# ikt-luh/Demo-Learned-Point-Cloud-Compression

Hardware: AMD Instinct MI355X
Metric: point-cloud frames/sec encode+decode @1M pts (higher is better)
Workload: dtype f32

## Files before the change

### demo-learned-point-cloud-compression_amd/csrc/codec.hip

```cpp
#include "common.h"

#include <string.h>

#include <algorithm>
#include <atomic>
#include <chrono>
#include <deque>
#include <exception>
#include <new>
#include <map>
#include <memory>
#include <string>
#include <condition_variable>
#include <functional>
#include <mutex>
#include <thread>
#include <vector>

namespace {

double now_s() {
  return std::chrono::duration<double>(std::chrono::steady_clock::now().time_since_epoch()).count();
}

// ... 1868 lines not shown
    slots.resize((size_t)n_frames);
    for (int f = 0; f < n_frames; ++f) {
      const int32_t pl = r.be32();
      for (int s = 0; s < 3; ++s) ks[s].push_back(r.be32());
      slots[f] = {r.bytes(pl), pl};
      PCC_REQUIRE(!r.bad, PCC_E_STREAM, "pcc_decode_gop: truncated container");
    }
    if (!v1 && len - r.pos >= 8 && memcmp(h_in + r.pos, "PCSK", 4) == 0) {
      Reader t{h_in + r.pos + 4, len - r.pos - 4};
      const int32_t cnt = t.be32();
      bool ok = cnt >= 1 && cnt <= 63 && (int64_t)cnt * 16 <= t.len - t.pos;
      for (int k = 0; ok && k < cnt; ++k) {
        const int64_t i = t.be32();
        const uint64_t hi = (uint32_t)t.be32(), lo = (uint32_t)t.be32();
        const int64_t w = t.be32();
        ok = !t.bad && i > (sk_idx.empty() ? 0 : sk_idx.back()) && i < (int64_t)ny_hdr * cy && w >= 2 && w * 4 <= ylen &&
             ((hi << 32) | lo) >= ((uint64_t)1 << 31);
        sk_idx.push_back(i);
        sk_state.push_back((hi << 32) | lo);
        sk_word.push_back(w);
      }
      if (!ok) sk_idx.clear();
    }
    return PCC_OK;
  }
  int check_sizes() {
    fn.assign((size_t)n_frames, 0);
    fdepth.assign((size_t)n_frames, 0);
    for (int f = 0; f < n_frames; ++f) {
      int32_t org[3];
      PCC_TRY(pcc_octree_peek(slots[f].p, slots[f].len, &fn[f], &fdepth[f], org));
      PCC_REQUIRE(fn[f] >= 0 && fn[f] <= ((int64_t)slots[f].len + 64) * 4096, PCC_E_STREAM,
                  "pcc_decode_gop: frame %d announces %lld points in a %d-byte blob", f, (long long)fn[f], slots[f].len);
      if (fn[f] > 0) {
        const int d = fdepth[f];
        PCC_REQUIRE(d >= 1 && d <= 13, PCC_E_STREAM, "pcc_decode_gop: frame %d: octree depth %d", f, d);
        for (int a = 0; a < 3; ++a) {
          const int64_t biased = (int64_t)org[a] + 4096;
          PCC_REQUIRE(biased >= 0 && biased + ((int64_t)1 << d) <= 8192 && (biased & (((int64_t)1 << d) - 1)) == 0,
                      PCC_E_STREAM, "pcc_decode_gop: frame %d: octree origin %d (axis %d) is not on the 2^%d grid", f,
                      org[a], a, d);
        }
      }
      ny += fn[f];
    }
    PCC_REQUIRE(ny == ny_hdr, PCC_E_STREAM, "pcc_decode_gop: container says N_y=%d, geometry gives %lld", ny_hdr,
                (long long)ny);
    PCC_REQUIRE(nz_hdr <= ny_hdr, PCC_E_STREAM, "pcc_decode_gop: container says N_z=%d > N_y=%d", nz_hdr, ny_hdr);
    PCC_REQUIRE(ny_hdr <= kMaxLatentRows, PCC_E_STREAM, "pcc_decode_gop: container says N_y=%d, this build decodes at most %lld",
                ny_hdr, (long long)kMaxLatentRows);
    return PCC_OK;
  }
  void start_z_job() {
    zsym.resize((size_t)std::max<int64_t>((int64_t)nz_hdr * cz, 1));
    cd->workers.run(0, [this]() {
      if (nz_hdr == 0) return;
      if (cd->eb_tables && cz <= 256) {
        std::vector<uint8_t> idx8((size_t)nz_hdr * cz);
        for (int c = 0; c < cz; ++c) memset(idx8.data() + (size_t)c * nz_hdr, c, (size_t)nz_hdr);
        z_rc = pcc_rans_decode8_gated(zstr, zlen, idx8.data(), (int64_t)nz_hdr * cz, eb_cdf->i32(), (int)eb_cdf->dims[1],
                                      eb_len->i32(), eb_off->i32(), (int)eb_cdf->dims[0], zsym.data(), nullptr, cd->eb_tables);
        if (z_rc != PCC_OK) z_err = pcc_last_error();
        return;
      }
      std::vector<int32_t> idx((size_t)nz_hdr * cz);
      for (int c = 0; c < cz; ++c) std::fill(idx.begin() + (size_t)c * nz_hdr, idx.begin() + (size_t)(c + 1) * nz_hdr, c);
      z_rc = pcc_rans_decode(zstr, zlen, idx.data(), (int64_t)nz_hdr * cz, eb_cdf->i32(), (int)eb_cdf->dims[1],
                             eb_len->i32(), eb_off->i32(), (int)eb_cdf->dims[0], zsym.data());
      if (z_rc != PCC_OK) z_err = pcc_last_error();
    });
  }
  int start_z() {
    eb_cdf = find(cd, "entropy_bottleneck.quantized_cdf");
    eb_len = find(cd, "entropy_bottleneck.cdf_length");
    eb_off = find(cd, "entropy_bottleneck.offset");
    PCC_REQUIRE(eb_cdf && eb_len && eb_off, PCC_E_ARG, "pcc_decode_gop: entropy_bottleneck tables missing");
    cd->workers.ensure(1);
    z_early = !v1 && (int64_t)nz_hdr * cz <= kEarlyZSymbols;
    if (z_early) start_z_job();
    if (!v1) return PCC_OK;
    int64_t zn = 0, yn = 0;
    PCC_TRY(pcc_rans_stream_info(zstr, zlen, &zn, &z_steps, &z_chunks));
    PCC_TRY(pcc_rans_stream_info(ystr, ylen, &yn, &y_steps, &y_chunks));
    PCC_REQUIRE(zn == (int64_t)nz_hdr * cz && yn == (int64_t)ny_hdr * cy, PCC_E_STREAM,
                "pcc_decode_gop: streams hold %lld / %lld symbols, header says %lld / %lld", (long long)yn, (long long)zn,
                (long long)ny_hdr * cy, (long long)nz_hdr * cz);
    d_status = (int32_t*)cd->pool.alloc(4);
    if (!d_status) return PCC_E_NOMEM;
    PCC_HIP(hipMemsetAsync(d_status, 0, 4, st));
    PCC_TRY(cd->pin_dec.ensure((size_t)ylen + (size_t)zlen + 512));
    memcpy(cd->pin_dec.p, zstr, (size_t)zlen);
    memcpy(cd->pin_dec.p + (((size_t)zlen + 255) & ~(size_t)255), ystr, (size_t)ylen);
    if ((int64_t)nz_hdr * cz <= kEarlyZSymbols) return z_stream_dev(&zsym_early);
    return PCC_OK;
  }
  int z_stream_dev(int32_t** zs) {
    const size_t zpad = ((size_t)zlen + 255) & ~(size_t)255;
    CODEC_ALLOC(d_str, uint8_t, zpad + (size_t)ylen + 256);
    if (!*zs) *zs = (int32_t*)cd->pool.alloc(sizeof(int32_t) * (size_t)(std::max<int64_t>((int64_t)nz_hdr, 1) * cz));
    if (!*zs) return PCC_E_NOMEM;
    PCC_HIP(hipMemcpyAsync(d_str, cd->pin_dec.p, zpad + (size_t)ylen, hipMemcpyHostToDevice, st));
    d_ystr = d_str + zpad;
    return pcc_rans_decode_dev(ctx, cd->eb_dev, d_str, zlen, (int64_t)nz_hdr * cz, z_steps, z_chunks, nullptr,
                               std::max<int64_t>(nz_hdr, 1), *zs, d_status);
  }
  int geometry() {
    std::vector<std::vector<int32_t>> fpts((size_t)n_frames);
    PCC_TRY(cd->pin_keys.ensure((size_t)std::max<int64_t>(ny, 1) * 16));
    int32_t* yc_h = (int32_t*)cd->pin_keys.p;
    std::vector<int64_t> frow((size_t)n_frames + 1, 0);
    for (int f = 0; f < n_frames; ++f) frow[(size_t)f + 1] = frow[(size_t)f] + fn[f];
    std::vector<PartJob> pjobs;
    std::vector<int> fpart0((size_t)n_frames, -1), fparts((size_t)n_frames, 0);
    for (int f = 0; f < n_frames; ++f) {
      if (fn[f] == 0 || slots[f].p[1] != 3) continue;
      int K = 0;
      const uint8_t* pp[16];
      int64_t pl[16];
      PCC_TRY(pcc_octree_parts(slots[f].p, slots[f].len, &K, pp, pl));
      int32_t org[3];
      PCC_TRY(pcc_octree_peek(slots[f].p, slots[f].len, nullptr, nullptr, org));
      fpart0[f] = (int)pjobs.size();
      fparts[f] = K;
      int64_t row = frow[(size_t)f];
      for (int k = 0; k < K; ++k) {
        int64_t n = 0;
        PCC_TRY(pcc_octree_peek(pp[k], pl[k], &n, nullptr, nullptr));
        pjobs.push_back({f, k, pp[k], pl[k], n, row, {org[0], org[1], org[2]}});
        row += n;
      }
    }
    constexpr int kPartThreads = 8;
    const int nj = (int)pjobs.size();
    if (nj > 0) cd->workers.ensure(kPartThreads);
    for (int j0 = 0; j0 < nj; j0 += kPartThreads) {
      const int j1 = std::min(nj, j0 + kPartThreads);
      for (int j = j0 + 1; j < j1; ++j) cd->workers.run(j - j0, [&pjobs, yc_h, j]() { run_part_job(pjobs[(size_t)j], yc_h); });
      run_part_job(pjobs[(size_t)j0], yc_h);
      cd->workers.wait_range(1, kPartThreads);
    }
    for (const PartJob& pj : pjobs)
      if (pj.rc != PCC_OK) {
        pcc_set_error("pcc_decode_gop (geometry, frame %d part %d): %s", pj.f, pj.k, pj.err.c_str());
        return pj.rc;
      }
    bool out_of_range = false;
    for (int f = 0; f < n_frames; ++f) {
      if (fn[f] == 0) continue;
      int64_t level_n[16];
      if (slots[f].p[1] == 3) {
        for (int L = 0; L < 16; ++L) level_n[L] = 0;
        bool any = false;
        uint64_t last = 0;
        int64_t total = 0;
        for (int k = 0; k < fparts[f]; ++k) {
          const PartJob& pj = pjobs[(size_t)(fpart0[f] + k)];
          out_of_range |= pj.out_of_range;
          if (pj.out.cells.empty()) continue;
          PCC_REQUIRE(!any || (pj.out.cells.front() >> 6) > (last >> 6), PCC_E_STREAM,
                      "pcc_decode_gop: frame %d: part %d begins inside or in front of the cell the part before it ends in", f, k);
          any = true;
          last = pj.out.cells.back();
          total += (int64_t)pj.out.cells.size();
          for (int L = 0; L < 16; ++L) level_n[L] += pj.out.level_n[L];
        }
        PCC_REQUIRE(total == fn[f], PCC_E_STREAM, "pcc_decode_gop: frame %d decoded %lld points, announced %lld", f, (long long)total,
                    (long long)fn[f]);
      } else {
        if (slots[f].p[1] == 2) {
          int64_t n2 = 0;
          fpts[f].resize((size_t)(3 * fn[f]));
          PCC_TRY(pcc_octree2_decode(ctx, slots[f].p, slots[f].len, nullptr, fpts[f].data(), fn[f], &n2, level_n));
        } else {
          PCC_TRY(pcc_octree_unpack_vec(slots[f].p, slots[f].len, &fpts[f], level_n));
        }
        PCC_REQUIRE((int64_t)fpts[f].size() == 3 * fn[f], PCC_E_STREAM, "pcc_decode_gop: frame %d decoded %zu points, announced %lld",
                    f, fpts[f].size() / 3, (long long)fn[f]);
        out_of_range |= put_leaf_rows(fpts[f].data(), fn[f], f, yc_h + 4 * frow[(size_t)f]);
      }
      const int depth = fdepth[f];
      n16 += depth >= 1 ? level_n[depth - 1] : 1;
      n32 += depth >= 2 ? level_n[depth - 2] : 1;
      n_batch = f + 1;
    }
    if (!z_early && !v1) start_z_job();
    PCC_REQUIRE(!out_of_range && n_batch <= 65535, PCC_E_RANGE, "pcc_decode_gop: decoded coordinate out of range");
    return PCC_OK;
  }
  int z_decode() {
    std::vector<int64_t> y_level_n(2, 0);
    CODEC_ALLOC(yc, int32_t, 4 * std::max<int64_t>(ny, 1));
    CODEC_ALLOC(keys, uint64_t, std::max<int64_t>(ny, 1));
    CODEC_ALLOC(flag, int32_t, 1);
    CODEC_ALLOC(perm, uint32_t, std::max<int64_t>(ny, 1));
    if (ny > 0) {
      PCC_HIP(hipMemcpyAsync(yc, cd->pin_keys.p, (size_t)ny * 16, hipMemcpyHostToDevice, st));
      PCC_HIP(hipMemsetAsync(flag, 0, 4, st));
      PCC_TRY(pcc_morton_keys(ctx, yc, ny, keys, flag));
      PCC_TRY(pcc_sort_pairs(ctx, keys, perm, ny, 0));
      y_level_n[0] = n16;
      y_level_n[1] = n32;
    }
    ycs = new_set(cd, keys, ny, 8, std::max(n_batch, 1));
    if (ny > 0) ycs->down_counts = y_level_n;
    PCC_TRY(down_of(cd, ycs));
    PCC_TRY(down_of(cd, ycs->down));
    CS* zcs = ycs->down->down;
    View zv;
    PCC_TRY(view_of(cd, zcs, &zv));
    PCC_REQUIRE(zcs->n == nz_hdr, PCC_E_STREAM, "pcc_decode_gop: container says N_z=%d, coordinates give %lld", nz_hdr,
                (long long)zcs->n);
    PCC_TRY(view_of(cd, ycs, &yv));
    {
      CS *a_cs, *pre_cs;
      PCC_TRY(up_of(cd, zcs, &a_cs));
      PCC_TRY(up_of(cd, a_cs, &pre_cs));
      PCC_TRY(h_s_book_at(cd, pre_cs, ycs, yv, &hs_book));
    }
    cd->workers.wait_all();
    if (z_rc != PCC_OK) {
      pcc_set_error("pcc_decode_gop (z stream): %s", z_err.c_str());
      return z_rc;
    }
    const int64_t nz = zcs->n;
    CODEC_ALLOC(zsym_d_own, int32_t, std::max<int64_t>(nz, 1) * cz);
    int32_t* zsym_d = zsym_d_own;
    CODEC_ALLOC(rows, float, std::max<int64_t>(nz, 1) * cz);
    if (v1) {
      if (zsym_early)
        zsym_d = zsym_early;
      else
        PCC_TRY(z_stream_dev(&zsym_d));
      if (nz > 0) PCC_TRY(pcc_factorized_dequant(ctx, zsym_d, nz, cz, cd->dev["entropy_bottleneck.medians"], rows));
    } else if (nz > 0) {
      PCC_TRY(cd->pin_zsym.ensure((size_t)nz * cz * 4));
      memcpy(cd->pin_zsym.p, zsym.data(), (size_t)nz * cz * 4);
      PCC_HIP(hipMemcpyAsync(zsym_d, cd->pin_zsym.p, (size_t)nz * cz * 4, hipMemcpyHostToDevice, st));
      PCC_TRY(pcc_factorized_dequant(ctx, zsym_d, nz, cz, cd->dev["entropy_bottleneck.medians"], rows));
    }
    float* zf;
    PCC_TRY(rows_to_tensor(cd, zv, rows, cz, &zf));
    z_hat = {zcs, zf, cz};
    return PCC_OK;
  }
  int y_decode() {
    float* params;
    PCC_TRY(h_s_out_at(cd, gp, ycs, yv, &params, hs_book));
    float* scale_d;
    const double q_dec[2] = {qg, qa};
    PCC_TRY(scale_rows_dev(cd, 1, q_dec, 1, &scale_d));
    const Tensor* tab = find(cd, "gaussian_conditional.scale_table");
    const Tensor *gc_cdf = find(cd, "gaussian_conditional.quantized_cdf"), *gc_len = find(cd, "gaussian_conditional.cdf_length"),
                 *gc_off = find(cd, "gaussian_conditional.offset");
    const Tensor* ab = find(cd, "entropy_model.offsets_ab");
    PCC_REQUIRE(tab && gc_cdf && gc_len && gc_off && ab, PCC_E_ARG, "pcc_decode_gop: gaussian_conditional tables missing");
    const int64_t tot = (int64_t)cy * ny;
    CODEC_ALLOC(idx8, uint8_t, std::max<int64_t>(tot, 1));
    CODEC_ALLOC(sym_d, int32_t, std::max<int64_t>(tot, 1));
    CODEC_ALLOC(rows, float, std::max<int64_t>(tot, 1));
    if (ny > 0 && v1) {
      PCC_TRY(pcc_gaussian_indexes8(ctx, params, ny, cy, scale_d, cd->dev["gaussian_conditional.scale_table"],
                                    (int)tab->dims[0], idx8));
      PCC_TRY(pcc_rans_decode_dev(ctx, cd->gc_dev, d_ystr, ylen, tot, y_steps, y_chunks, idx8, 1, sym_d, d_status));
      PCC_TRY(pcc_gaussian_dequant(ctx, sym_d, params, ny, cy, scale_d, tab->f32()[0], ab->f32()[0], ab->f32()[1], rows));
    } else if (ny > 0) {
      PCC_TRY(pcc_gaussian_indexes8(ctx, params, ny, cy, scale_d, cd->dev["gaussian_conditional.scale_table"],
                                    (int)tab->dims[0], idx8));
      PCC_TRY(cd->pin_yidx.ensure((size_t)tot));
      PCC_TRY(cd->pin_dec.ensure((size_t)tot * 4));
      PCC_HIP(hipMemcpyAsync(cd->pin_yidx.p, idx8, (size_t)tot, hipMemcpyDeviceToHost, st));
      PCC_HIP(hipStreamSynchronize(st));
      {
        CS* c0;
        int32_t* nbr0;
        PCC_TRY(up_of(cd, ycs, &c0));
        PCC_TRY(nbr27_of(cd, pcc_conv_up_fused() ? ycs : c0, &nbr0));
      }
      bool decoded = false;
      if (!sk_idx.empty() && cd->gc_tables) {
        const int pieces = (int)sk_idx.size() + 1;
        std::vector<int> prc((size_t)pieces, PCC_OK);
        std::vector<uint64_t> end_x((size_t)pieces, 0);
        std::vector<int64_t> end_w((size_t)pieces, 0);
        auto piece = [&](int k) {
          const int64_t lo = k == 0 ? 0 : sk_idx[k - 1], hi = k == pieces - 1 ? tot : sk_idx[k];
          prc[k] = pcc_rans_decode8_range(ystr, ylen, cd->pin_yidx.p, tot, gc_cdf->i32(), (int)gc_cdf->dims[1], gc_len->i32(),
                                          gc_off->i32(), (int)gc_cdf->dims[0], (int32_t*)cd->pin_dec.p, cd->gc_tables, lo, hi,
                                          k == 0 ? 0 : sk_state[k - 1], k == 0 ? 0 : sk_word[k - 1], &end_x[k], &end_w[k]);
        };
        {
          WorkersGuard wait_pieces{&cd->workers};
          cd->workers.ensure(pieces - 1);
          for (int k = 1; k < pieces; ++k) cd->workers.run(k - 1, [&piece, k]() { piece(k); });
          piece(0);
        }
        decoded = true;
        for (int k = 0; k < pieces; ++k) {
          decoded &= prc[k] == PCC_OK;
          if (k + 1 < pieces) decoded &= end_x[k] == sk_state[k] && end_w[k] == sk_word[k];
        }
        if (decoded)
          PCC_HIP(hipMemcpyAsync(sym_d, cd->pin_dec.p, (size_t)tot * 4, hipMemcpyHostToDevice, st));
      }
      const int n_chunks = tot >= (1 << 16) ? 4 : 1;
      std::vector<int64_t> bound((size_t)n_chunks);
      for (int c = 0; c < n_chunks; ++c) bound[c] = c == n_chunks - 1 ? tot : (tot * (c + 1) / n_chunks) & ~(int64_t)63;
      struct UpUser {
        const int64_t* bound;
        const uint8_t* host;
        int32_t* dev;
        hipStream_t st;
        bool failed;
      } up{bound.data(), cd->pin_dec.p, sym_d, st, false};
      PccRansGate gate{n_chunks, bound.data(),
                       [](void* u, int c) {
                         UpUser* g = (UpUser*)u;
                         const int64_t lo = c == 0 ? 0 : g->bound[c - 1], hi = g->bound[c];
                         if (hi > lo && hipMemcpyAsync(g->dev + lo, g->host + (size_t)lo * 4, (size_t)(hi - lo) * 4,
                                                       hipMemcpyHostToDevice, g->st) != hipSuccess)
                           g->failed = true;
                       },
                       &up};
      if (!decoded)
        PCC_TRY(pcc_rans_decode8_gated(ystr, ylen, cd->pin_yidx.p, tot, gc_cdf->i32(), (int)gc_cdf->dims[1],
                                       gc_len->i32(), gc_off->i32(), (int)gc_cdf->dims[0], (int32_t*)cd->pin_dec.p,
                                       &gate, cd->gc_tables));
      PCC_REQUIRE(!up.failed, PCC_E_HIP, "pcc_decode_gop: hipMemcpyAsync of decoded symbols failed");
      PCC_TRY(pcc_gaussian_dequant(ctx, sym_d, params, ny, cy, scale_d, tab->f32()[0], ab->f32()[0], ab->f32()[1], rows));
    }
    float* yf;
    PCC_TRY(rows_to_tensor(cd, yv, rows, cy, &yf));
    y_hat = {ycs, yf, cy};
    return PCC_OK;
  }
  int synthesis(const PackedDst* dst) {
    Feat h = y_hat;
    const int nb = h.cs->n_batch;
    {
      const std::vector<int64_t>* o0;
      PCC_TRY(offsets_of(cd, h.cs, &o0));
    }
    const float* rgb_cand = nullptr;
    bool tail = false;
    uint64_t* tail_pkeys = nullptr;
    int tail_shift = 0;
    for (int j = 0; j < 3; ++j) {
      const std::string uname = "g_s.up" + std::to_string(j);
      const std::string cname = "g_s.conv" + std::to_string(j), oname = "g_s.occ" + std::to_string(j);
      const float *w, *b, *hw, *hb;
      const Tensor *tw, *thw;
      PCC_TRY(wb(cd, cname, &w, &b, &tw));
      PCC_TRY(wb(cd, oname, &hw, &hb, &thw));
      const int cin = (int)tw->dims[1], cout = (int)tw->dims[2];
      const bool fused = pcc_conv_up_fused() && cin == 32 && cout == 32 && cd->dev.count(uname + ".weight#perm");
      Feat u;
      PCC_TRY(up2(cd, uname, h, 1, &u, fused));
      const int64_t nu = u.cs->n;
      const Tensor* tcol = find(cd, "g_s.color.weight");
      const bool with_rgb = fused && j == 2 && nu > 0 && tcol && tcol->dims.size() == 2 && tcol->dims[0] == 32 &&
                            tcol->dims[1] == 3;
      float* feats = nullptr;
      if (!with_rgb) {
        feats = (float*)cd->pool.alloc(sizeof(float) * (size_t)(std::max<int64_t>(nu, 1) * cout));
        if (!feats) return PCC_E_NOMEM;
      }
      CODEC_ALLOC(logits, float, std::max<int64_t>(nu, 1));
      if (with_rgb) {
        int32_t* pn;
        PCC_TRY(nbr27_of(cd, h.cs, &pn));
        CODEC_ALLOC(rgb_all, float, nu * 3);
        rgb_cand = rgb_all;
        PCC_TRY(pcc_sparse_conv_head_up_perm_rgb(ctx, u.f, h.cs->n, pn, h.cs->n, w, b, 1, hw, hb, logits,
                                                 cd->dev["g_s.color.weight"], cd->dev["g_s.color.bias"], rgb_all));
      } else if (fused && nu > 0) {
        int32_t* pn;
        PCC_TRY(nbr27_of(cd, h.cs, &pn));
        PCC_TRY(pcc_sparse_conv_head_up_perm(ctx, u.f, h.cs->n, pn, h.cs->n, w, b, 1, feats, hw, hb, logits));
      } else if (nu == 0) {
      } else {
        int32_t* nbr;
        PCC_TRY(nbr27_of(cd, u.cs, &nbr));
        PCC_TRY(pcc_sparse_conv_head(ctx, u.f, nu, nbr, 27, nu, nu, w, b, cin, cout, 1, feats, hw, hb, logits));
      }
      const std::vector<int64_t>* offs;
      PCC_TRY(offsets_of(cd, u.cs, &offs));
      std::vector<int64_t> kj((size_t)nb), new_offs(1, 0);
      for (int f = 0; f < nb; ++f) {
        const int64_t want = f < (int)ks[j].size() ? ks[j][f] : 0;
        kj[f] = std::max<int64_t>(0, std::min<int64_t>(want, (*offs)[f + 1] - (*offs)[f]));
        new_offs.push_back(new_offs.back() + kj[f]);
      }
      CODEC_ALLOC(keep, uint32_t, std::max<int64_t>(nu, 1));
      const int64_t n_keep = new_offs.back();
      int32_t* keep_remap = nullptr;
      if (nu > 0 && j + 1 < 3) {
        keep_remap = (int32_t*)cd->pool.alloc(sizeof(int32_t) * (size_t)nu);
        if (!keep_remap) return PCC_E_NOMEM;
      }
      if (nu > 0) PCC_TRY(pcc_topk_prune_map(ctx, logits, nu, nb, offs->data(), kj.data(), keep, nullptr, keep_remap));
      CODEC_ALLOC(pkeys, uint64_t, std::max<int64_t>(n_keep, 1));
      CODEC_ALLOC(pf, float, std::max<int64_t>(n_keep, 1) * cout);
      const bool in_place = cout == 32;
      tail = with_rgb && in_place && n_keep > 0 && !u.cs->keys && u.cs->gen_parent;
      if (tail) {
        PCC_TRY(keys_of(cd, u.cs->gen_parent, &tail_pkeys));
        tail_shift = 3 * log2i(u.cs->stride);
        pkeys = nullptr;
      } else if (n_keep > 0) {
        if (!u.cs->keys && u.cs->gen_parent) {
          uint64_t* pk;
          PCC_TRY(keys_of(cd, u.cs->gen_parent, &pk));
          PCC_TRY(pcc_up_coords_rows(ctx, pk, u.cs->gen_parent->n, 3 * log2i(u.cs->stride), keep, n_keep, pkeys));
        } else {
          PCC_TRY(pcc_gather_rows(ctx, u.cs->keys, keep, n_keep, 8, pkeys));
        }
        if (!in_place) PCC_TRY(pcc_gather_rows(ctx, feats, keep, n_keep, 4 * cout, pf));
      }
      CS* ps = new_set(cd, pkeys, n_keep, u.cs->stride, nb);
      ps->offsets = new_offs;
      ps->subset_of = u.cs;
      ps->keep = keep;
      ps->keep_remap = keep_remap;
      h = {ps, in_place ? feats : pf, cout, in_place ? keep : nullptr};
    }
    {
      const float *w, *b;
      const Tensor* tw;
      PCC_TRY(wb(cd, "g_s.color", &w, &b, &tw));
      const int64_t nr = h.cs->n;
      CODEC_ALLOC(rgb, float, std::max<int64_t>(nr, 1) * 3);
      CODEC_ALLOC(coords, int32_t, std::max<int64_t>(nr, 1) * 4);
      cd->rec_xyz16 = nullptr;
      cd->rec_rgbp = nullptr;
      if (nr > 0 && tail && rgb_cand && h.rows) {
        if (dst && nr <= dst->cap) {
          CODEC_ALLOC(xyz16, int16_t, nr * 3);
          CODEC_ALLOC(rgbp, float, nr * 3);
          cd->rec_xyz16 = xyz16;
          cd->rec_rgbp = rgbp;
        }
        hipLaunchKernelGGL(k_decode_tail, dim3((unsigned)((nr + 255) / 256)), dim3(256), 0, st, (const uint64_t*)tail_pkeys,
                           tail_shift, h.rows, nr, rgb_cand, (int4*)coords, rgb, cd->rec_xyz16, cd->rec_rgbp);
        PCC_CHECK_LAUNCH();
      } else if (nr > 0) {
        if (rgb_cand && h.rows)
          PCC_TRY(pcc_gather_rows(ctx, rgb_cand, h.rows, nr, 12, rgb));
        else if (h.rows && (int)tw->dims[0] == 32 && (int)tw->dims[1] <= 8)
          PCC_TRY(pcc_linear_gather(ctx, h.f, h.rows, nr, w, b, (int)tw->dims[1], 0, rgb));
        else if (h.rows) {
          CODEC_ALLOC(pf, float, nr * h.c);
          PCC_TRY(pcc_gather_rows(ctx, h.f, h.rows, nr, 4 * h.c, pf));
          PCC_TRY(pcc_linear(ctx, pf, nr, w, b, (int)tw->dims[0], (int)tw->dims[1], 0, rgb));
        } else
          PCC_TRY(pcc_linear(ctx, h.f, nr, w, b, (int)tw->dims[0], (int)tw->dims[1], 0, rgb));
        uint64_t* hkeys;
        PCC_TRY(keys_of(cd, h.cs, &hkeys));
        PCC_TRY(pcc_keys_to_coords(ctx, hkeys, nr, coords));
      }
      cd->rec_coords = coords;
      cd->rec_i16 = true;
      cd->rec_colors = rgb;
      cd->rec_n = nr;
      cd->rec_offsets = h.cs->offsets;
    }
    return finish(dst);
  }
  int finish(const PackedDst* dst) {
    if (v1) {
      PCC_TRY(cd->pin_flag.ensure(64));
      PCC_HIP(hipMemcpyAsync(cd->pin_flag.p, d_status, 4, hipMemcpyDeviceToHost, st));
    }
    if (dst && cd->rec_n > 0) {
      PCC_REQUIRE(cd->rec_n <= dst->cap && dst->points && dst->colors, PCC_E_ARG,
                  "pcc_decode_gop_packed: %lld points decoded, destination holds %lld", (long long)cd->rec_n,
                  (long long)dst->cap);
      PCC_TRY(queue_packed(cd, dst->points, dst->colors));
    }
    PCC_TRY(pcc_sync(ctx));
    if (dst && cd->rec_n > 0) {
      cd->workers.wait_all();
      PCC_REQUIRE(cd->widen_status.load() == 0, PCC_E_HIP, "pcc_decode_gop_packed: wait for the points' copy failed");
    }
    if (v1 && *(volatile int32_t*)cd->pin_flag.p != 0) {
      cd->rec_n = 0;
      cd->rec_offsets.clear();
      pcc_set_error("pcc_decode_gop: malformed interleaved rANS stream (status %d)", *(int32_t*)cd->pin_flag.p);
      return PCC_E_STREAM;
    }
    return PCC_OK;
  }
};

}

static int decode_gop_impl(pcc_codec* cd, const uint8_t* h_in, int64_t len, pcc_cloud_info* h_info,
                           double* h_stage_s, const PackedDst* dst = nullptr) {
  PCC_REQUIRE(cd && cd->ctx, PCC_E_ARG, "pcc_decode_gop: null codec");
  PCC_REQUIRE(h_in && len >= 36 && h_info, PCC_E_STREAM, "pcc_decode_gop: container shorter than its header");
  PCC_TRY(begin_call(cd));
  cd->rec_n = 0;
  cd->rec_offsets.clear();
  cd->rec_i16 = false;
  cd->rec_xyz16 = nullptr;
  cd->rec_rgbp = nullptr;
  DecodeCall c(cd);
  PCC_TRY(timed(&c.ts[0], [&] { return c.parse(h_in, len); }));
  PCC_TRY(c.check_sizes());
  WorkersGuard z_job{&cd->workers};
  PCC_TRY(c.start_z());
  PCC_TRY(timed(&c.ts[1], [&] { return c.geometry(); }));
  PCC_TRY(timed(&c.ts[2], [&] { return c.z_decode(); }));
  PCC_TRY(timed(&c.ts[3], [&] { return h_s_up(cd, c.z_hat, &c.gp); }));
  PCC_TRY(timed(&c.ts[4], [&] { return c.y_decode(); }));
  PCC_TRY(timed(&c.ts[5], [&] { return c.synthesis(dst); }));
  h_info->n_points = cd->rec_n;
  h_info->n_frames = c.n_frames;
  h_info->n_offsets = (int32_t)cd->rec_offsets.size();
  h_info->h_offsets = cd->rec_offsets.data();
  h_info->d_coords = cd->rec_coords;
  h_info->d_colors = cd->rec_colors;
  h_info->q_g = c.qg;
  h_info->q_a = c.qa;
  if (h_stage_s) memcpy(h_stage_s, c.ts, 6 * sizeof(double));
  return PCC_OK;
}

template <class F>
static int no_throw(const char* name, int code, F&& call) {
  try {
    return call();
  } catch (const std::bad_alloc&) {
    pcc_set_error("%s: out of host memory", name);
    return PCC_E_NOMEM;
  } catch (const std::exception& e) {
    pcc_set_error("%s: %s", name, e.what());
    return code;
  }
}

static int frame_table(const char* name, const void* const* pts, int points_i16, const void* const* cols, int colors_f64,
                       const int64_t* h_n, int n_frames, FrameTab* t) {
  memset(t, 0, sizeof(*t));
  t->nf = n_frames;
  t->pts_i16 = points_i16 ? 1 : 0;
  t->cols_f64 = colors_f64 ? 1 : 0;
  for (int f = 0; f < n_frames; ++f) {
    PCC_REQUIRE(h_n[f] >= 0 && (h_n[f] == 0 || (pts[f] && cols[f])), PCC_E_ARG, "%s: frame %d: n=%lld or null arrays", name,
                f, (long long)h_n[f]);
    t->pts[f] = pts[f];
    t->cols[f] = cols[f];
    t->off[f + 1] = t->off[f] + h_n[f];
  }
  PCC_REQUIRE(t->off[n_frames] < ((int64_t)1 << 32), PCC_E_ARG, "%s: %lld points", name, (long long)t->off[n_frames]);
  return PCC_OK;
}

extern "C" int pcc_encode_gop(pcc_codec* cd, const int32_t* d_coords, const float* d_feats, int64_t n,
                              int n_frames, const double* h_q, int n_q, pcc_buf* h_out, int64_t* h_k,
                              double* h_stage_s) {
  return no_throw("pcc_encode_gop", PCC_E_ARG,
                  [&] { return encode_gop_impl(cd, d_coords, d_feats, n, n_frames, h_q, n_q, h_out, h_k, h_stage_s); });
}

extern "C" int pcc_encode_gop_frames(pcc_codec* cd, const void* const* h_d_points, int points_i16,
                                     const void* const* h_d_colors, int colors_f64, const int64_t* h_n, int n_frames,
                                     const double* h_q, int n_q, pcc_buf* h_out, int64_t* h_k, double* h_stage_s) {
  PCC_REQUIRE(h_d_points && h_d_colors && h_n && n_frames >= 1, PCC_E_ARG, "pcc_encode_gop_frames: null frame table");
  PCC_REQUIRE(n_frames <= PCC_MAX_FRAMES_ARG, PCC_E_ARG,
              "pcc_encode_gop_frames: %d frames, at most %d per call (concatenate and use pcc_encode_gop)", n_frames,
              PCC_MAX_FRAMES_ARG);
  FrameTab t;
  PCC_TRY(frame_table("pcc_encode_gop_frames", h_d_points, points_i16, h_d_colors, colors_f64, h_n, n_frames, &t));
  return no_throw("pcc_encode_gop_frames", PCC_E_ARG, [&] {
    return encode_gop_impl(cd, nullptr, nullptr, t.off[n_frames], n_frames, h_q, n_q, h_out, h_k, h_stage_s, &t);
  });
}

extern "C" int pcc_encode_gop_host_frames(pcc_codec* cd, const void* const* h_points, int points_i16,
                                          const void* const* h_colors, int colors_f64, const int64_t* h_n, int n_frames,
                                          const double* h_q, int n_q, pcc_buf* h_out, int64_t* h_k, double* h_stage_s) {
  PCC_REQUIRE(h_points && h_colors && h_n && n_frames >= 1, PCC_E_ARG, "pcc_encode_gop_host_frames: null frame table");
  PCC_REQUIRE(n_frames <= PCC_MAX_FRAMES_ARG, PCC_E_ARG, "pcc_encode_gop_host_frames: %d frames, at most %d per call",
              n_frames, PCC_MAX_FRAMES_ARG);
  FrameTab t;
  PCC_TRY(frame_table("pcc_encode_gop_host_frames", h_points, points_i16, h_colors, colors_f64, h_n, n_frames, &t));
  const HostFrames host{h_points, h_colors};
  return no_throw("pcc_encode_gop_host_frames", PCC_E_ARG, [&] {
    return encode_gop_impl(cd, nullptr, nullptr, t.off[n_frames], n_frames, h_q, n_q, h_out, h_k, h_stage_s, &t, &host);
  });
}

extern "C" int pcc_decode_gop(pcc_codec* cd, const uint8_t* h_in, int64_t len, pcc_cloud_info* h_info,
                              double* h_stage_s) {
  return no_throw("pcc_decode_gop", PCC_E_STREAM, [&] { return decode_gop_impl(cd, h_in, len, h_info, h_stage_s); });
}

extern "C" int pcc_decode_gop_packed(pcc_codec* cd, const uint8_t* h_in, int64_t len, int32_t* points, float* colors,
                                     int64_t cap_points, pcc_cloud_info* h_info, double* h_stage_s) {
  PCC_REQUIRE(points && colors && cap_points >= 0, PCC_E_ARG, "pcc_decode_gop_packed: null destination");
  const PackedDst dst{points, colors, cap_points};
  return no_throw("pcc_decode_gop_packed", PCC_E_STREAM, [&] { return decode_gop_impl(cd, h_in, len, h_info, h_stage_s, &dst); });
}

extern "C" int pcc_container_points(const uint8_t* h_in, int64_t len, int64_t* h_n_points, int32_t* h_n_frames) {
  PCC_REQUIRE(h_in && len >= 36 && h_n_points, PCC_E_STREAM, "pcc_container_points: container shorter than its header");
  Reader r{h_in, len};
  const int32_t word0 = r.be32();
  const int32_t n_frames = (int32_t)((uint32_t)word0 & 0x00FFFFFFu);
  (void)r.be_f64();
// ... 119 lines not shown
```

### demo-learned-point-cloud-compression_amd/csrc/rans_host.cpp

```cpp
#include <stdint.h>
#include <string.h>
#include <stdio.h>
#include <algorithm>
#include <memory>
#include <thread>
#include <vector>
#include "../../include/pcc.h"
#include "rans_gate.h"

void pcc_set_error(const char* fmt, ...);

namespace {

constexpr uint32_t kPrecision = 16;
constexpr uint32_t kBypassBits = 4;
constexpr uint32_t kMaxBypass = (1u << kBypassBits) - 1;
constexpr uint64_t kRansL = 1ull << 31;

struct Enc {
  uint64_t x;
  uint32_t* ptr;
  uint32_t* floor;
  bool overflow;

  inline void emit(uint32_t w) {
    if (ptr == floor) { overflow = true; return; }
    *--ptr = w;
  }
  inline void put(const struct EncSym& e);
  inline void put_bits(uint32_t val) {
    const uint32_t freq = 1u << (16 - kBypassBits);
    const uint64_t x_max = ((kRansL >> 16) << 32) * freq;
    if (x >= x_max) { emit((uint32_t)x); x >>= 32; }
    x = (x << kBypassBits) | val;
  }
};

struct EncSym {
  uint64_t rcp;
  uint64_t x_max;
  uint32_t bias;
  uint32_t cmpl;
  uint32_t freq;
  uint32_t rs;
};
inline void Enc::put(const EncSym& e) {
  if (x >= e.x_max) { emit((uint32_t)x); x >>= 32; }
  const uint64_t q = (uint64_t)(((unsigned __int128)e.rcp * x) >> 64) >> e.rs;
  x = x + e.bias + q * e.cmpl;
}

inline int n_nibbles(uint32_t raw) {
  int nb = 0;
  while ((raw >> (nb * kBypassBits)) != 0) ++nb;
  return nb;
}

struct EncTables {
  std::vector<int32_t> base;
  std::vector<EncSym> ent;
};

int build_enc_tables(const int32_t* cdfs, int pitch, const int32_t* sizes, int n_cdf, EncTables* t, char* err,
                     size_t errlen) {
  t->base.assign((size_t)n_cdf + 1, 0);
  for (int c = 0; c < n_cdf; ++c) {
    if (sizes[c] < 2 || sizes[c] > pitch) {
      snprintf(err, errlen, "rans encode: cdf %d has length %d", c, sizes[c]);
      return PCC_E_ARG;
    }
    t->base[c + 1] = t->base[c] + sizes[c] - 1;
  }
  t->ent.resize((size_t)t->base[n_cdf]);
  for (int c = 0; c < n_cdf; ++c) {
    const int32_t* cdf = cdfs + (int64_t)c * pitch;
    for (int v = 0; v < sizes[c] - 1; ++v) {
      EncSym& e = t->ent[(size_t)t->base[c] + v];
      const int64_t f = (int64_t)cdf[v + 1] - cdf[v];
      e.freq = (f >= 1 && f <= 65536) ? (uint32_t)f : 0u;
      e.bias = (uint32_t)cdf[v];
      e.cmpl = (1u << kPrecision) - e.freq;
      if (e.freq < 2) {
        e.rcp = ~0ull;
        e.rs = 0;
        e.bias += (1u << kPrecision) - 1;
      } else {
        uint32_t shift = 0;
        while (e.freq > (1u << shift)) ++shift;
        e.rcp = (uint64_t)((((unsigned __int128)1 << (shift + 63)) + e.freq - 1) / e.freq);
        e.rs = shift - 1;
      }
      e.x_max = ((kRansL >> kPrecision) << 32) * (uint64_t)e.freq;
    }
  }
  return PCC_OK;
}

template <typename SymT, typename IdxT>
int encode_stream(const SymT* sym, const IdxT* idx, int64_t n, const int32_t* cdfs, int pitch,
                  const int32_t* sizes, const int32_t* offsets, int n_cdf, uint8_t* out, int64_t cap,
                  int64_t* len, char* err, size_t errlen, const PccRansGate* gate = nullptr,
                  const EncTables* pre = nullptr, PccRansSeek* seek = nullptr) {
  size_t buf_words = (size_t)(n / 2 + n / 8) + 1024;
  std::unique_ptr<uint32_t[]> buf(new uint32_t[buf_words]);
  EncTables local;
  if (!pre) {
    const int rc = build_enc_tables(cdfs, pitch, sizes, n_cdf, &local, err, errlen);
    if (rc != PCC_OK) return rc;
    pre = &local;
  }
  const std::vector<int32_t>& base = pre->base;
  const std::vector<EncSym>& ent = pre->ent;
  for (int attempt = 0; attempt < 3; ++attempt) {
    Enc e;
    e.x = kRansL;
    e.floor = buf.get();
    e.ptr = buf.get() + buf_words;
    e.overflow = false;
    const int n_chunks = gate ? gate->n_chunks : 1;
    int sk = seek ? seek->n - 1 : -1;
    while (sk >= 0 && seek->index[sk] >= n) --sk;
    for (int ch = 0; ch < n_chunks; ++ch) {
    const int64_t c_hi = (ch == 0 ? n : gate->bound[ch - 1]) - 1, c_lo = gate ? gate->bound[ch] : 0;
    if (gate) gate->fn(gate->user, ch);
    for (int64_t i_hi = c_hi; i_hi >= c_lo;) {
    const int64_t i_lo = (sk >= 0 && seek->index[sk] > c_lo) ? std::min<int64_t>(seek->index[sk], i_hi + 1) : c_lo;
    for (int64_t i = i_hi; i >= i_lo; --i) {
      const int32_t ci = (int32_t)idx[i];
      if ((uint32_t)ci >= (uint32_t)n_cdf) {
        snprintf(err, errlen, "rans encode: index %d out of range at %lld", ci, (long long)i);
        return PCC_E_ARG;
      }
      const int32_t max_value = sizes[ci] - 2;
      int32_t value = (int32_t)sym[i] - offsets[ci];
      if ((uint32_t)value >= (uint32_t)max_value) {
        uint32_t raw;
        if (value < 0) raw = (uint32_t)(-2 * (int64_t)value - 1);
        else raw = (uint32_t)(2 * ((int64_t)value - max_value));
        value = max_value;
        const int nb = n_nibbles(raw);
        for (int j = nb - 1; j >= 0; --j) e.put_bits((raw >> (j * kBypassBits)) & kMaxBypass);
        const int full = nb / (int)kMaxBypass;
        e.put_bits((uint32_t)(nb - full * (int)kMaxBypass));
        for (int j = 0; j < full; ++j) e.put_bits(kMaxBypass);
      }
      const EncSym& es = ent[(size_t)base[ci] + value];
      if (es.freq == 0) {
        snprintf(err, errlen, "rans encode: zero frequency (cdf %d, value %d)", ci, value);
        return PCC_E_ARG;
      }
      e.put(es);
    }
    while (sk >= 0 && seek->index[sk] >= i_lo && seek->index[sk] > 0) {
      seek->state[sk] = e.x;
      seek->word[sk] = (int64_t)((buf.get() + buf_words) - e.ptr);
      --sk;
    }
    i_hi = i_lo - 1;
    }
    }
    e.emit((uint32_t)(e.x >> 32));
    e.emit((uint32_t)(e.x >> 0));
    if (e.overflow) {
      buf_words = (size_t)n * 12 + 1024;
      buf.reset(new uint32_t[buf_words]);
      continue;
    }
    const int64_t nbytes = (int64_t)((buf.get() + buf_words) - e.ptr) * 4;
    if (nbytes > cap) {
      snprintf(err, errlen, "rans encode: output needs %lld bytes, capacity %lld", (long long)nbytes,
               (long long)cap);
      return PCC_E_NOMEM;
    }
    memcpy(out, e.ptr, (size_t)nbytes);
    *len = nbytes;
    if (seek) {
      const int64_t total = nbytes / 4;
      for (int k = 0; k < seek->n; ++k) {
        if (seek->index[k] <= 0 || seek->index[k] >= n) { seek->state[k] = 0; seek->word[k] = 0; continue; }
        seek->word[k] = total - seek->word[k];
      }
    }
    return PCC_OK;
  }
  snprintf(err, errlen, "rans encode: internal buffer overflow");
  return PCC_E_NOMEM;
}

template <typename SymT, typename IdxT>
int encode_multi(const SymT* h_sym, const IdxT* h_idx, int64_t n, int n_streams, const int32_t* h_cdfs,
                 int cdf_pitch, const int32_t* h_sizes, const int32_t* h_offsets, int n_cdf, uint8_t* h_out,
                 int64_t cap_each, int64_t* h_lens, const char* who) {
  if (n_streams < 1 || n_streams > 64 || !h_lens || n < 0 || (n > 0 && (!h_sym || !h_idx)) || !h_cdfs ||
      !h_sizes || !h_offsets || !h_out || cdf_pitch < 2 || n_cdf < 1) {
    pcc_set_error("%s: bad argument", who);
    return PCC_E_ARG;
  }
  std::vector<int> rc((size_t)n_streams, PCC_OK);
  std::vector<std::vector<char>> errs((size_t)n_streams, std::vector<char>(256, 0));
  auto work = [&](int s) {
    rc[s] = encode_stream(h_sym + (int64_t)s * n, h_idx + (int64_t)s * n, n, h_cdfs, cdf_pitch, h_sizes,
                          h_offsets, n_cdf, h_out + (int64_t)s * cap_each, cap_each, &h_lens[s],
                          errs[s].data(), errs[s].size());
  };
  std::vector<std::thread> th;
  for (int s = 1; s < n_streams; ++s) th.emplace_back(work, s);
  work(0);
  for (auto& t : th) t.join();
  for (int s = 0; s < n_streams; ++s)
    if (rc[s] != PCC_OK) {
      pcc_set_error("%s stream %d: %s", who, s, errs[s].data());
      return rc[s];
    }
  return PCC_OK;
}

struct DecTab {
  const uint32_t* sym;
  const uint64_t* lut;
  int32_t max_value, offset;
};
constexpr int kLutBits = 10;

struct DecTables {
  std::vector<DecTab> tabs;
  std::vector<uint64_t> luts;
  std::vector<uint32_t> syms;
};

int build_dec_tables(const int32_t* h_cdfs, int cdf_pitch, const int32_t* h_sizes, const int32_t* h_offsets, int n_cdf,
                     const uint8_t* used , DecTables* t, const char* who) {
  t->tabs.assign((size_t)n_cdf, DecTab{nullptr, nullptr, 0, 0});
  t->luts.assign((size_t)n_cdf << kLutBits, 0ull);
  size_t total = 0;
  for (int c = 0; c < n_cdf; ++c) {
    if (used && !used[c]) continue;
    if (h_sizes[c] < 2 || h_sizes[c] > cdf_pitch) {
      pcc_set_error("%s: cdf %d has length %d", who, c, h_sizes[c]);
      return PCC_E_ARG;
    }
    total += (size_t)h_sizes[c] - 1;
  }
  t->syms.assign(total + 1, 0u);
  total = 0;
  for (int c = 0; c < n_cdf; ++c) {
    if (used && !used[c]) continue;
    const int32_t* cdf = h_cdfs + (int64_t)c * cdf_pitch;
    const int size = h_sizes[c];
    uint32_t* sy = t->syms.data() + total;
    for (int v = 0; v < size - 1; ++v) sy[v] = ((uint32_t)(cdf[v + 1] - cdf[v]) << 16) | ((uint32_t)cdf[v] & 0xFFFFu);
    uint64_t* lut = t->luts.data() + ((size_t)c << kLutBits);
    int s = 0;
    for (int b = 0; b < (1 << kLutBits); ++b) {
      const int lo = b << (16 - kLutBits), hi = lo + (1 << (16 - kLutBits));
      while (s + 1 < size - 1 && cdf[s + 1] <= lo) ++s;
      const bool cut = s + 1 < size - 1 && cdf[s + 1] < hi;
      lut[b] = (uint64_t)sy[s] | ((uint64_t)s << 32) | ((uint64_t)cut << 63);
    }
    t->tabs[c].sym = sy;
    t->tabs[c].lut = lut;
    t->tabs[c].max_value = size - 2;
    t->tabs[c].offset = h_offsets[c];
    total += (size_t)size - 1;
  }
  return PCC_OK;
}

struct DecPos {
  uint64_t x;
  int64_t word;
};
template <typename IdxT>
int decode_stream(const uint8_t* h_in, int64_t len, const IdxT* h_idx, int64_t n, const int32_t* h_cdfs,
                  int cdf_pitch, const int32_t* h_sizes, const int32_t* h_offsets, int n_cdf, int32_t* h_sym,
                  const char* who, const PccRansGate* gate = nullptr, const DecTables* pre = nullptr,
                  int64_t r_lo = 0, int64_t r_hi = -1, const DecPos* from = nullptr, DecPos* to = nullptr) {
  if (!h_in || len < 8 || n < 0 || (n > 0 && (!h_idx || !h_sym)) || !h_cdfs || !h_sizes || !h_offsets ||
      cdf_pitch < 2 || n_cdf < 1) {
    pcc_set_error("%s: bad argument (len=%lld)", who, (long long)len);
    return len < 8 ? PCC_E_STREAM : PCC_E_ARG;
  }
  const bool ranged = from != nullptr;
  if (r_hi < 0) r_hi = n;
  if (ranged && (gate || r_lo < 0 || r_lo > r_hi || r_hi > n || from->word < 2 || from->word * 4 > len)) {
    pcc_set_error("%s: bad range", who);
    return PCC_E_ARG;
  }
  {
    uint32_t worst = 0;
    for (int64_t i = r_lo; i < r_hi; ++i) worst = std::max(worst, (uint32_t)(int32_t)h_idx[i]);
    if (r_hi > r_lo && worst >= (uint32_t)n_cdf) {
      for (int64_t i = r_lo; i < r_hi; ++i)
        if ((uint32_t)(int32_t)h_idx[i] >= (uint32_t)n_cdf) {
          pcc_set_error("%s: index %d out of range at %lld", who, (int32_t)h_idx[i], (long long)i);
          return PCC_E_ARG;
        }
    }
  }
  DecTables local;
  if (!pre) {
    std::vector<uint8_t> used((size_t)n_cdf, 0);
    for (int64_t i = r_lo; i < r_hi; ++i) used[(size_t)(int32_t)h_idx[i]] = 1;
    const int rc = build_dec_tables(h_cdfs, cdf_pitch, h_sizes, h_offsets, n_cdf, used.data(), &local, who);
    if (rc != PCC_OK) return rc;
    pre = &local;
  }
  const std::vector<DecTab>& tabs = pre->tabs;
  const uint8_t* p = h_in;
  const uint8_t* const end = h_in + len;
  auto word = [&](bool& bad) -> uint32_t {
    if (end - p < 4) { bad = true; return 0; }
    uint32_t w;
    memcpy(&w, p, 4);
    p += 4;
    return w;
  };
  bool bad = false;
  uint64_t x;
  if (ranged) {
    x = from->x;
    p = h_in + from->word * 4;
  } else {
    x = word(bad);
    x |= (uint64_t)word(bad) << 32;
  }
  const int n_chunks = gate ? gate->n_chunks : 1;
  for (int ch = 0; ch < n_chunks; ++ch) {
  const int64_t i_lo = gate ? (ch == 0 ? 0 : gate->bound[ch - 1]) : r_lo, i_hi = gate ? gate->bound[ch] : r_hi;
  for (int64_t i = i_lo; i < i_hi; ++i) {
    const DecTab& t = tabs[(size_t)(int32_t)h_idx[i]];
    const uint32_t cum = (uint32_t)(x & 0xFFFFu);
    const uint64_t l = t.lut[cum >> (16 - kLutBits)];
    int32_t s = (int32_t)((l >> 32) & 0xFFFFu);
    uint32_t e = (uint32_t)l;
    if (__builtin_expect((int64_t)l < 0, 0)) {
      while (s < t.max_value && (t.sym[s + 1] & 0xFFFFu) <= cum) ++s;
      e = t.sym[s];
    }
    x = (uint64_t)(e >> 16) * (x >> kPrecision) + cum - (e & 0xFFFFu);
    if (x < kRansL) x = (x << 32) | word(bad);
    int32_t value = s;
    if (__builtin_expect(value == t.max_value, 0)) {
      auto get_bits = [&]() -> uint32_t {
        const uint32_t v = (uint32_t)(x & kMaxBypass);
        x >>= kBypassBits;
        if (x < kRansL) x = (x << 32) | word(bad);
        return v;
      };
      int32_t val = (int32_t)get_bits();
      int32_t n_bypass = val;
      while (val == (int32_t)kMaxBypass && !bad) {
        val = (int32_t)get_bits();
        n_bypass += val;
      }
      if (n_bypass > 8) {
        pcc_set_error("%s: corrupt escape at symbol %lld", who, (long long)i);
        return PCC_E_STREAM;
      }
      uint32_t raw = 0;
      for (int j = 0; j < n_bypass; ++j) raw |= get_bits() << (j * kBypassBits);
      value = (int32_t)(raw >> 1);
      if (raw & 1u) value = -value - 1;
      else value += t.max_value;
    }
    h_sym[i] = value + t.offset;
  }
  if (gate && !bad) gate->fn(gate->user, ch);
  }
  if (bad) {
    pcc_set_error("%s: truncated stream", who);
    return PCC_E_STREAM;
  }
  if (to) {
    to->x = x;
    to->word = (int64_t)(p - h_in) / 4;
  }
  return PCC_OK;
}

}

static bool gate_ok(const PccRansGate* g, int64_t n, bool descending) {
  if (!g) return true;
  if (g->n_chunks < 1 || !g->bound || !g->fn) return false;
  for (int c = 0; c < g->n_chunks; ++c) {
    const int64_t b = g->bound[c], prev = c == 0 ? (descending ? n : 0) : g->bound[c - 1];
    if (b < 0 || b > n || (descending ? b > prev : b < prev)) return false;
  }
  return g->bound[g->n_chunks - 1] == (descending ? 0 : n);
}

struct PccRansTables {
  EncTables enc;
  DecTables dec;
};

PccRansTables* pcc_rans_tables_build(const int32_t* h_cdfs, int cdf_pitch, const int32_t* h_sizes,
                                     const int32_t* h_offsets, int n_cdf) {
  if (!h_cdfs || !h_sizes || !h_offsets || cdf_pitch < 2 || n_cdf < 1) {
    pcc_set_error("pcc_rans_tables_build: bad argument");
    return nullptr;
  }
  std::unique_ptr<PccRansTables> t(new PccRansTables);
  char err[256] = {0};
  if (build_enc_tables(h_cdfs, cdf_pitch, h_sizes, n_cdf, &t->enc, err, sizeof(err)) != PCC_OK) {
    pcc_set_error("pcc_rans_tables_build: %s", err);
    return nullptr;
  }
  if (build_dec_tables(h_cdfs, cdf_pitch, h_sizes, h_offsets, n_cdf, nullptr, &t->dec, "pcc_rans_tables_build") != PCC_OK)
    return nullptr;
  return t.release();
}

void pcc_rans_tables_free(PccRansTables* t) { delete t; }

int pcc_rans_encode16_gated(const int16_t* h_sym, const uint8_t* h_idx, int64_t n, const int32_t* h_cdfs,
                            int cdf_pitch, const int32_t* h_sizes, const int32_t* h_offsets, int n_cdf,
                            uint8_t* h_out, int64_t cap, int64_t* h_len, const PccRansGate* gate,
                            const PccRansTables* tables) {
  if (!h_len || n < 0 || (n > 0 && (!h_sym || !h_idx)) || !h_cdfs || !h_sizes || !h_offsets || !h_out ||
      cdf_pitch < 2 || n_cdf < 1 || !gate_ok(gate, n, true)) {
    pcc_set_error("pcc_rans_encode16_gated: bad argument");
    return PCC_E_ARG;
  }
  char err[256] = {0};
  const int rc = encode_stream(h_sym, h_idx, n, h_cdfs, cdf_pitch, h_sizes, h_offsets, n_cdf, h_out, cap, h_len, err,
                               sizeof(err), gate, tables ? &tables->enc : nullptr);
  if (rc != PCC_OK) pcc_set_error("pcc_rans_encode16_gated: %s", err);
  return rc;
}

int pcc_rans_encode16_seek(const int16_t* h_sym, const uint8_t* h_idx, int64_t n, const int32_t* h_cdfs,
                           int cdf_pitch, const int32_t* h_sizes, const int32_t* h_offsets, int n_cdf,
                           uint8_t* h_out, int64_t cap, int64_t* h_len, const PccRansGate* gate,
                           const PccRansTables* tables, PccRansSeek* seek) {
  if (!h_len || n < 0 || (n > 0 && (!h_sym || !h_idx)) || !h_cdfs || !h_sizes || !h_offsets || !h_out ||
      cdf_pitch < 2 || n_cdf < 1 || !gate_ok(gate, n, true)) {
    pcc_set_error("pcc_rans_encode16_seek: bad argument");
    return PCC_E_ARG;
  }
  if (seek)
    for (int k = 0; k < seek->n; ++k)
      if (!seek->index || !seek->state || !seek->word || (k > 0 && seek->index[k] < seek->index[k - 1])) {
        pcc_set_error("pcc_rans_encode16_seek: seek indexes must ascend");
        return PCC_E_ARG;
      }
  char err[256] = {0};
  const int rc = encode_stream(h_sym, h_idx, n, h_cdfs, cdf_pitch, h_sizes, h_offsets, n_cdf, h_out, cap, h_len, err,
                               sizeof(err), gate, tables ? &tables->enc : nullptr, seek);
  if (rc != PCC_OK) pcc_set_error("pcc_rans_encode16_seek: %s", err);
  return rc;
}

int pcc_rans_decode8_range(const uint8_t* h_in, int64_t len, const uint8_t* h_idx, int64_t n, const int32_t* h_cdfs,
                           int cdf_pitch, const int32_t* h_sizes, const int32_t* h_offsets, int n_cdf, int32_t* h_sym,
                           const PccRansTables* tables, int64_t i_lo, int64_t i_hi, uint64_t state_in, int64_t word_in,
                           uint64_t* state_out, int64_t* word_out) {
  if (!tables || !state_out || !word_out || !h_in || len < 8) {
    pcc_set_error("pcc_rans_decode8_range: bad argument");
    return PCC_E_ARG;
  }
  DecPos from{state_in, word_in}, to{0, 0};
  if (i_lo == 0 && word_in == 0) {
    uint32_t w[2];
    memcpy(w, h_in, 8);
    from.x = (uint64_t)w[0] | ((uint64_t)w[1] << 32);
    from.word = 2;
  }
  const int rc = decode_stream(h_in, len, h_idx, n, h_cdfs, cdf_pitch, h_sizes, h_offsets, n_cdf, h_sym,
                               "pcc_rans_decode8_range", nullptr, &tables->dec, i_lo, i_hi, &from, &to);
  *state_out = to.x;
  *word_out = to.word;
  return rc;
}

int pcc_rans_decode8_gated(const uint8_t* h_in, int64_t len, const uint8_t* h_idx, int64_t n, const int32_t* h_cdfs,
                           int cdf_pitch, const int32_t* h_sizes, const int32_t* h_offsets, int n_cdf,
                           int32_t* h_sym, const PccRansGate* gate, const PccRansTables* tables) {
  if (!gate_ok(gate, n, false)) {
    pcc_set_error("pcc_rans_decode8_gated: bad chunk table");
    return PCC_E_ARG;
  }
  return decode_stream(h_in, len, h_idx, n, h_cdfs, cdf_pitch, h_sizes, h_offsets, n_cdf, h_sym,
                       "pcc_rans_decode8", gate, tables ? &tables->dec : nullptr);
}

extern "C" int pcc_rans_encode(const int32_t* h_sym, const int32_t* h_idx, int64_t n,
                               const int32_t* h_cdfs, int cdf_pitch, const int32_t* h_sizes,
                               const int32_t* h_offsets, int n_cdf, uint8_t* h_out, int64_t cap,
                               int64_t* h_len) {
  return encode_multi(h_sym, h_idx, n, 1, h_cdfs, cdf_pitch, h_sizes, h_offsets, n_cdf, h_out, cap, h_len,
                      "pcc_rans_encode");
}

extern "C" int pcc_rans_encode_multi(const int32_t* h_sym, const int32_t* h_idx, int64_t n,
                                     int n_streams, const int32_t* h_cdfs, int cdf_pitch,
                                     const int32_t* h_sizes, const int32_t* h_offsets, int n_cdf,
                                     uint8_t* h_out, int64_t cap_each, int64_t* h_lens) {
  return encode_multi(h_sym, h_idx, n, n_streams, h_cdfs, cdf_pitch, h_sizes, h_offsets, n_cdf, h_out,
                      cap_each, h_lens, "pcc_rans_encode_multi");
}

extern "C" int pcc_rans_encode_multi16(const int16_t* h_sym, const uint8_t* h_idx, int64_t n,
                                       int n_streams, const int32_t* h_cdfs, int cdf_pitch,
                                       const int32_t* h_sizes, const int32_t* h_offsets, int n_cdf,
                                       uint8_t* h_out, int64_t cap_each, int64_t* h_lens) {
  return encode_multi(h_sym, h_idx, n, n_streams, h_cdfs, cdf_pitch, h_sizes, h_offsets, n_cdf, h_out,
                      cap_each, h_lens, "pcc_rans_encode_multi16");
}

extern "C" int pcc_rans_decode(const uint8_t* h_in, int64_t len, const int32_t* h_idx, int64_t n,
                               const int32_t* h_cdfs, int cdf_pitch, const int32_t* h_sizes,
                               const int32_t* h_offsets, int n_cdf, int32_t* h_sym) {
  return decode_stream(h_in, len, h_idx, n, h_cdfs, cdf_pitch, h_sizes, h_offsets, n_cdf, h_sym,
                       "pcc_rans_decode");
}

extern "C" int pcc_rans_encode_seek(const int32_t* h_sym, const int32_t* h_idx, int64_t n, const int32_t* h_cdfs,
                                    int cdf_pitch, const int32_t* h_sizes, const int32_t* h_offsets, int n_cdf,
                                    uint8_t* h_out, int64_t cap, int64_t* h_len, const int64_t* h_seek_index, int n_seek,
                                    uint64_t* h_seek_state, int64_t* h_seek_word) {
  if (!h_len || n < 0 || (n > 0 && (!h_sym || !h_idx)) || !h_cdfs || !h_sizes || !h_offsets || !h_out || cdf_pitch < 2 ||
      n_cdf < 1 || n_seek < 0 || (n_seek > 0 && (!h_seek_index || !h_seek_state || !h_seek_word))) {
    pcc_set_error("pcc_rans_encode_seek: bad argument");
    return PCC_E_ARG;
  }
  for (int k = 1; k < n_seek; ++k)
    if (h_seek_index[k] < h_seek_index[k - 1]) {
      pcc_set_error("pcc_rans_encode_seek: seek indexes must ascend");
      return PCC_E_ARG;
    }
  PccRansSeek seek{n_seek, h_seek_index, h_seek_state, h_seek_word};
  char err[256] = {0};
  const int rc = encode_stream(h_sym, h_idx, n, h_cdfs, cdf_pitch, h_sizes, h_offsets, n_cdf, h_out, cap, h_len, err,
                               sizeof(err), nullptr, nullptr, n_seek ? &seek : nullptr);
  if (rc != PCC_OK) pcc_set_error("pcc_rans_encode_seek: %s", err);
  return rc;
}

extern "C" int pcc_rans_decode_range(const uint8_t* h_in, int64_t len, const int32_t* h_idx, int64_t n,
                                     const int32_t* h_cdfs, int cdf_pitch, const int32_t* h_sizes, const int32_t* h_offsets,
                                     int n_cdf, int32_t* h_sym, int64_t i_lo, int64_t i_hi, uint64_t state_in,
                                     int64_t word_in, uint64_t* h_state_out, int64_t* h_word_out) {
  if (!h_state_out || !h_word_out || !h_in || len < 8) {
    pcc_set_error("pcc_rans_decode_range: bad argument");
    return len < 8 && h_in ? PCC_E_STREAM : PCC_E_ARG;
  }
  DecPos from{state_in, word_in}, to{0, 0};
  if (i_lo == 0 && word_in == 0) {
    uint32_t w[2];
    memcpy(w, h_in, 8);
    from.x = (uint64_t)w[0] | ((uint64_t)w[1] << 32);
    from.word = 2;
  }
  const int rc = decode_stream(h_in, len, h_idx, n, h_cdfs, cdf_pitch, h_sizes, h_offsets, n_cdf, h_sym,
                               "pcc_rans_decode_range", nullptr, nullptr, i_lo, i_hi, &from, &to);
  *h_state_out = to.x;
  *h_word_out = to.word;
  return rc;
}

extern "C" int pcc_rans_decode8(const uint8_t* h_in, int64_t len, const uint8_t* h_idx, int64_t n,
                                const int32_t* h_cdfs, int cdf_pitch, const int32_t* h_sizes,
                                const int32_t* h_offsets, int n_cdf, int32_t* h_sym) {
  return decode_stream(h_in, len, h_idx, n, h_cdfs, cdf_pitch, h_sizes, h_offsets, n_cdf, h_sym,
                       "pcc_rans_decode8");
}
```

Before: 116.7.

## Use geometric upload chunks and a struct-packed per-CDF rANS decode LUT

```diff
diff --git a/demo-learned-point-cloud-compression_amd/csrc/codec.hip b/demo-learned-point-cloud-compression_amd/csrc/codec.hip
--- a/demo-learned-point-cloud-compression_amd/csrc/codec.hip
+++ b/demo-learned-point-cloud-compression_amd/csrc/codec.hip
@@ -2194,9 +2194,9 @@
         if (decoded)
           PCC_HIP(hipMemcpyAsync(sym_d, cd->pin_dec.p, (size_t)tot * 4, hipMemcpyHostToDevice, st));
       }
-      const int n_chunks = tot >= (1 << 16) ? 4 : 1;
+      const int n_chunks = tot >= (1 << 16) ? 6 : 1;
       std::vector<int64_t> bound((size_t)n_chunks);
-      for (int c = 0; c < n_chunks; ++c) bound[c] = c == n_chunks - 1 ? tot : (tot * (c + 1) / n_chunks) & ~(int64_t)63;
+      for (int c = 0; c < n_chunks; ++c) bound[c] = c == n_chunks - 1 ? tot : (tot - (tot >> (c + 1))) & ~(int64_t)63;
       struct UpUser {
         const int64_t* bound;
         const uint8_t* host;
diff --git a/demo-learned-point-cloud-compression_amd/csrc/rans_host.cpp b/demo-learned-point-cloud-compression_amd/csrc/rans_host.cpp
--- a/demo-learned-point-cloud-compression_amd/csrc/rans_host.cpp
+++ b/demo-learned-point-cloud-compression_amd/csrc/rans_host.cpp
@@ -215,24 +215,48 @@
   return PCC_OK;
 }
 
+struct DecEnt {
+  uint16_t start, freq;
+  uint16_t sym;
+  uint16_t cut;
+};
+static_assert(sizeof(DecEnt) == 8, "one lookup entry is one 8-byte word");
 struct DecTab {
   const uint32_t* sym;
-  const uint64_t* lut;
+  const DecEnt* lut;
   int32_t max_value, offset;
-};
-constexpr int kLutBits = 10;
+  uint32_t shift;
+};
+constexpr int kLutMinBits = 6, kLutMaxBits = 10;
+#ifndef PCC_RANS_LUT_CUT
+#define PCC_RANS_LUT_CUT 0
+#endif
+constexpr uint32_t kLutCutBound = PCC_RANS_LUT_CUT;
 
 struct DecTables {
   std::vector<DecTab> tabs;
-  std::vector<uint64_t> luts;
+  std::vector<DecEnt> luts;
   std::vector<uint32_t> syms;
 };
+
+inline int cut_buckets(const int32_t* cdf, int size, int bits) {
+  const int w = 16 - bits;
+  int n = 0;
+  int64_t last = -1;
+  for (int v = 1; v < size - 1; ++v) {
+    const int64_t c = cdf[v];
+    if (c <= 0 || c >= 65536 || (c & ((1 << w) - 1)) == 0) continue;
+    n += (c >> w) != last;
+    last = c >> w;
+  }
+  return n;
+}
 
 int build_dec_tables(const int32_t* h_cdfs, int cdf_pitch, const int32_t* h_sizes, const int32_t* h_offsets, int n_cdf,
                      const uint8_t* used , DecTables* t, const char* who) {
-  t->tabs.assign((size_t)n_cdf, DecTab{nullptr, nullptr, 0, 0});
-  t->luts.assign((size_t)n_cdf << kLutBits, 0ull);
-  size_t total = 0;
+  t->tabs.assign((size_t)n_cdf, DecTab{nullptr, nullptr, 0, 0, 0});
+  std::vector<int> bits((size_t)n_cdf, kLutMaxBits);
+  size_t total = 0, lut_total = 0;
   for (int c = 0; c < n_cdf; ++c) {
     if (used && !used[c]) continue;
     if (h_sizes[c] < 2 || h_sizes[c] > cdf_pitch) {
@@ -240,28 +264,38 @@
       return PCC_E_ARG;
     }
     total += (size_t)h_sizes[c] - 1;
+    for (int b = kLutMinBits; b < kLutMaxBits && kLutCutBound; ++b)
+      if (((uint32_t)cut_buckets(h_cdfs + (int64_t)c * cdf_pitch, h_sizes[c], b) << (16 - b)) <= kLutCutBound) {
+        bits[c] = b;
+        break;
+      }
+    lut_total += (size_t)1 << bits[c];
   }
   t->syms.assign(total + 1, 0u);
-  total = 0;
+  t->luts.assign(lut_total, DecEnt{0, 0, 0, 0});
+  total = lut_total = 0;
   for (int c = 0; c < n_cdf; ++c) {
     if (used && !used[c]) continue;
     const int32_t* cdf = h_cdfs + (int64_t)c * cdf_pitch;
     const int size = h_sizes[c];
     uint32_t* sy = t->syms.data() + total;
     for (int v = 0; v < size - 1; ++v) sy[v] = ((uint32_t)(cdf[v + 1] - cdf[v]) << 16) | ((uint32_t)cdf[v] & 0xFFFFu);
-    uint64_t* lut = t->luts.data() + ((size_t)c << kLutBits);
+    DecEnt* lut = t->luts.data() + lut_total;
+    const int shift = 16 - bits[c];
     int s = 0;
-    for (int b = 0; b < (1 << kLutBits); ++b) {
-      const int lo = b << (16 - kLutBits), hi = lo + (1 << (16 - kLutBits));
+    for (int b = 0; b < (1 << bits[c]); ++b) {
+      const int lo = b << shift, hi = lo + (1 << shift);
       while (s + 1 < size - 1 && cdf[s + 1] <= lo) ++s;
       const bool cut = s + 1 < size - 1 && cdf[s + 1] < hi;
-      lut[b] = (uint64_t)sy[s] | ((uint64_t)s << 32) | ((uint64_t)cut << 63);
+      lut[b] = DecEnt{(uint16_t)(sy[s] & 0xFFFFu), (uint16_t)(sy[s] >> 16), (uint16_t)s, (uint16_t)cut};
     }
     t->tabs[c].sym = sy;
     t->tabs[c].lut = lut;
     t->tabs[c].max_value = size - 2;
     t->tabs[c].offset = h_offsets[c];
+    t->tabs[c].shift = (uint32_t)shift;
     total += (size_t)size - 1;
+    lut_total += (size_t)1 << bits[c];
   }
   return PCC_OK;
 }
@@ -330,21 +364,25 @@
   for (int64_t i = i_lo; i < i_hi; ++i) {
     const DecTab& t = tabs[(size_t)(int32_t)h_idx[i]];
     const uint32_t cum = (uint32_t)(x & 0xFFFFu);
-    const uint64_t l = t.lut[cum >> (16 - kLutBits)];
-    int32_t s = (int32_t)((l >> 32) & 0xFFFFu);
-    uint32_t e = (uint32_t)l;
-    if (__builtin_expect((int64_t)l < 0, 0)) {
+    const DecEnt* const l = t.lut + (cum >> t.shift);
+    int32_t s = l->sym;
+    uint64_t freq = l->freq;
+    uint64_t rest = (uint64_t)cum - l->start;
+    if (__builtin_expect(l->cut != 0, 0)) {
       while (s < t.max_value && (t.sym[s + 1] & 0xFFFFu) <= cum) ++s;
-      e = t.sym[s];
-    }
-    x = (uint64_t)(e >> 16) * (x >> kPrecision) + cum - (e & 0xFFFFu);
+      const uint32_t e = t.sym[s];
+      freq = e >> 16;
+      rest = (uint64_t)cum - (e & 0xFFFFu);
+    }
+    x = freq * (x >> kPrecision) + rest;
     if (x < kRansL) x = (x << 32) | word(bad);
     int32_t value = s;
     if (__builtin_expect(value == t.max_value, 0)) {
+      uint64_t xe = x;
       auto get_bits = [&]() -> uint32_t {
-        const uint32_t v = (uint32_t)(x & kMaxBypass);
-        x >>= kBypassBits;
-        if (x < kRansL) x = (x << 32) | word(bad);
+        const uint32_t v = (uint32_t)(xe & kMaxBypass);
+        xe >>= kBypassBits;
+        if (xe < kRansL) xe = (xe << 32) | word(bad);
         return v;
       };
       int32_t val = (int32_t)get_bits();
@@ -362,6 +400,7 @@
       value = (int32_t)(raw >> 1);
       if (raw & 1u) value = -value - 1;
       else value += t.max_value;
+      x = xe;
     }
     h_sym[i] = value + t.offset;
   }
```

New measurement: 111.7. -4.3%, worse.
